# mrlooi/PoseCNN

Measured on AMD Instinct MI355X. Metric: frames/sec 640x480x21-class Hough-vote+RoI+ADD-loss, 1/2/4/8 MI355X, higher is better.
Workload: dtype f32 (FC GEMMs: exact 3-way split-bf16 x6 MFMA, products within 2^-24, fp32 accumulate: fp32-faithful)

## Files before the change

### include/posecnn_hip.h

```cpp
#ifndef POSECNN_HIP_H
#define POSECNN_HIP_H

#include <stddef.h>
#include <stdint.h>

#ifdef __cplusplus
extern "C" {
#endif

#define PCNN_OK 0
#define PCNN_EINVAL 1
#define PCNN_EHIP 2
#define PCNN_ECAPACITY 3

#define PCNN_MAX_ROI 128

int pcnn_abi_version(void);
const char* pcnn_strerror(int code);

int pcnn_set_completion_event(void* event);
int pcnn_completion_event_pending(void);

size_t pcnn_hough_voting_workspace_size(int B, int H, int W, int C, int skip_pixels, float vote_thr);

// ... 36 lines not shown
                           float scale_b, int B, int C, const float* rois, int R_cap, int roi_stride,
                           int batch_base, const int32_t* num_rois_dev, int pooled_h, int pooled_w, float* top_sum,
                           int32_t* argmax_a, int32_t* argmax_b, void* stream);

int pcnn_roi_pool_fwd_pair_px(const float* data_a, int Ha, int Wa, float scale_a, const float* data_b, int Hb,
                              int Wb, float scale_b, int B, int C, const float* rois, int R_cap, int roi_stride,
                              int batch_base, const int32_t* num_rois_dev, int pooled_h, int pooled_w,
                              float* top_sum, uint16_t* argmax_a, uint16_t* argmax_b, void* stream);

size_t pcnn_roi_pool_bwd_workspace_size(int B, int R_cap);

int pcnn_roi_pool_bwd_form(int B, int H, int W, int C, int layout, int pool_channel, int pooled_h, int pooled_w,
                           int R_cap, int px);

int pcnn_roi_pool_bwd(const float* top_diff, const int32_t* argmax, int B, int H, int W, int C, int layout,
                      const float* rois, int R_cap, int roi_stride, int batch_base, const int32_t* num_rois_dev,
                      float spatial_scale, int pooled_h, int pooled_w, int pool_channel, float* bottom_diff,
                      void* workspace, size_t workspace_bytes, void* stream);

int pcnn_roi_pool_bwd_px(const float* top_diff, const uint16_t* argmax_px, int B, int H, int W, int C,
                         const float* rois, int R_cap, int roi_stride, int batch_base, const int32_t* num_rois_dev,
                         float spatial_scale, int pooled_h, int pooled_w, float* bottom_diff, void* workspace,
                         size_t workspace_bytes, void* stream);

size_t pcnn_add_loss_workspace_size(int R_cap, int C, int P);
size_t pcnn_add_loss_stats_offset(int R_cap, int C, int P);

int pcnn_add_loss_fwd(const float* pred, const float* target, const float* weight, const float* points,
                      const float* symmetry, int R_cap, const int32_t* num_rois_dev, int C, int P, float margin,
                      int loss_norm_rows, const int32_t* loss_norm_rows_dev, float* loss, float* bottom_diff,
                      void* workspace, size_t workspace_bytes, void* stream);

int pcnn_add_loss_prep(const float* weight, const float* symmetry, int R_cap, const int32_t* num_rois_dev, int C,
                       int P, void* workspace, size_t workspace_bytes, void* stream);
int pcnn_add_loss_fwd_prepared(const float* pred, const float* target, const float* weight, const float* points,
                               const float* symmetry, int R_cap, const int32_t* num_rois_dev, int C, int P,
                               float margin, int loss_norm_rows, const int32_t* loss_norm_rows_dev, float* loss,
                               float* bottom_diff, void* workspace, size_t workspace_bytes, void* stream);

int pcnn_add_loss_fwd_head_bwd(const float* pred, const float* target, const float* weight, const float* points,
                               const float* symmetry, int R_cap, const int32_t* num_rois_dev, int C, int P,
                               float margin, int loss_norm_rows, const int32_t* loss_norm_rows_dev,
                               float* bottom_diff, void* workspace, size_t workspace_bytes, const float* tanh_out,
                               const float* d_pred_scale, float* d_y8, void* stream);
int pcnn_add_loss_total(int R_cap, const int32_t* num_rois_dev, int C, int P, const void* workspace,
                        size_t workspace_bytes, float* loss, void* stream);
// ... 197 lines not shown
```

### posecnn_amd/_lib.py

```python
import ctypes
import os
import threading

import torch

_HERE = os.path.dirname(os.path.abspath(__file__))
LIB_PATH = os.environ.get("POSECNN_HIP_LIB") or os.path.join(_HERE, "libposecnn_hip.so")

_lib = None
_lock = threading.Lock()

c_int = ctypes.c_int
c_float = ctypes.c_float
c_size_t = ctypes.c_size_t
c_void_p = ctypes.c_void_p

_SIGS = {
    "pcnn_abi_version": (c_int, []),
    "pcnn_strerror": (ctypes.c_char_p, [c_int]),
    "pcnn_set_completion_event": (c_int, [c_void_p]),
    "pcnn_completion_event_pending": (c_int, []),
    "pcnn_hough_voting_workspace_size": (c_size_t, [c_int, c_int, c_int, c_int, c_int, c_float]),
    "pcnn_hough_voting": (c_int, [c_void_p, c_void_p, c_void_p, c_void_p, c_int, c_void_p, c_int, c_int, c_int,
                                  c_int, c_int, c_int, c_int, c_int, c_float, c_int, c_float, c_float, c_int,
# ... 3 lines not shown
                                       c_int, c_int, c_int, c_int, c_int, c_int, c_int, c_float, c_int, c_float,
                                       c_float, c_int, c_void_p, c_void_p, c_void_p, c_void_p, c_void_p, c_void_p,
                                       c_int, c_void_p, c_void_p, c_size_t, c_void_p]),
    "pcnn_hough_voting_compact": (c_int, [c_void_p, c_void_p, c_void_p, c_void_p, c_int, c_void_p, c_int, c_int,
                                          c_int, c_int, c_int, c_int, c_int, c_int, c_float, c_int, c_float, c_float,
                                          c_int, c_void_p, c_void_p, c_void_p, c_void_p, c_void_p, c_void_p, c_int,
                                          c_void_p, c_void_p, c_size_t, c_void_p]),
    "pcnn_hough_voting_grad": (c_int, [c_void_p, c_void_p, c_int, c_int, c_int, c_int, c_void_p]),
    "pcnn_hough_voting_diag": (c_int, [c_void_p, c_int, c_int, c_int, c_int, c_int, c_float, c_void_p, c_void_p]),
    "pcnn_roi_pool_fwd": (c_int, [c_void_p, c_int, c_int, c_int, c_int, c_int, c_void_p, c_int, c_int, c_int,
                                  c_void_p, c_float, c_int, c_int, c_int, c_void_p, c_void_p, c_void_p]),
    "pcnn_roi_pool_fwd_accumulate": (c_int, [c_void_p, c_int, c_int, c_int, c_int, c_int, c_void_p, c_int, c_int,
                                             c_int, c_void_p, c_float, c_int, c_int, c_int, c_void_p, c_void_p, c_void_p]),
    "pcnn_roi_pool_fwd_pair": (c_int, [c_void_p, c_int, c_int, c_float, c_void_p, c_int, c_int, c_float, c_int, c_int,
                                       c_void_p, c_int, c_int, c_int, c_void_p, c_int, c_int, c_void_p, c_void_p,
                                       c_void_p, c_void_p]),
    "pcnn_roi_pool_fwd_pair_px": (c_int, [c_void_p, c_int, c_int, c_float, c_void_p, c_int, c_int, c_float, c_int,
                                          c_int, c_void_p, c_int, c_int, c_int, c_void_p, c_int, c_int, c_void_p,
                                          c_void_p, c_void_p, c_void_p]),
    "pcnn_roi_pool_bwd_workspace_size": (c_size_t, [c_int, c_int]),
    "pcnn_roi_pool_bwd_form": (c_int, [c_int, c_int, c_int, c_int, c_int, c_int, c_int, c_int, c_int, c_int]),
    "pcnn_roi_pool_bwd_px": (c_int, [c_void_p, c_void_p, c_int, c_int, c_int, c_int, c_void_p, c_int, c_int, c_int,
                                     c_void_p, c_float, c_int, c_int, c_void_p, c_void_p, c_size_t, c_void_p]),
    "pcnn_roi_pool_bwd": (c_int, [c_void_p, c_void_p, c_int, c_int, c_int, c_int, c_int, c_void_p, c_int, c_int,
                                  c_int, c_void_p, c_float, c_int, c_int, c_int, c_void_p, c_void_p, c_size_t, c_void_p]),
    "pcnn_add_loss_workspace_size": (c_size_t, [c_int, c_int, c_int]),
    "pcnn_add_loss_stats_offset": (c_size_t, [c_int, c_int, c_int]),
    "pcnn_add_loss_fwd": (c_int, [c_void_p, c_void_p, c_void_p, c_void_p, c_void_p, c_int, c_void_p, c_int, c_int,
                                  c_float, c_int, c_void_p, c_void_p, c_void_p, c_void_p, c_size_t, c_void_p]),
    "pcnn_add_loss_fwd_prepared": (c_int, [c_void_p, c_void_p, c_void_p, c_void_p, c_void_p, c_int, c_void_p, c_int, c_int,
                                  c_float, c_int, c_void_p, c_void_p, c_void_p, c_void_p, c_size_t, c_void_p]),
    "pcnn_add_loss_prep": (c_int, [c_void_p, c_void_p, c_int, c_void_p, c_int, c_int, c_void_p, c_size_t, c_void_p]),
    "pcnn_add_loss_fwd_head_bwd": (c_int, [c_void_p, c_void_p, c_void_p, c_void_p, c_void_p, c_int, c_void_p, c_int,
                                           c_int, c_float, c_int, c_void_p, c_void_p, c_void_p, c_size_t, c_void_p,
                                           c_void_p, c_void_p, c_void_p]),
    "pcnn_add_loss_total": (c_int, [c_int, c_void_p, c_int, c_int, c_void_p, c_size_t, c_void_p, c_void_p]),
    "pcnn_add_loss_bwd": (c_int, [c_void_p, c_void_p, c_int, c_void_p, c_int, c_void_p, c_void_p]),
    "pcnn_div_rn_check": (c_int, [c_void_p, c_float, c_int, c_int, c_void_p, c_void_p]),
    "pcnn_backproject_fwd": (c_int, [c_void_p, c_void_p, c_void_p, c_void_p, c_int, c_void_p, c_int, c_int, c_int,
                                     c_int, c_int, c_int, c_int, c_float, c_void_p, c_void_p, c_void_p, c_void_p]),
    "pcnn_backproject_bwd": (c_int, [c_void_p, c_void_p, c_void_p, c_int, c_int, c_int, c_int, c_int, c_int,
                                     c_void_p, c_void_p]),
    "pcnn_gemm_workspace_size": (c_size_t, [c_int, c_int, c_int, c_int, c_int]),
    "pcnn_gemm": (c_int, [c_int, c_int, c_int, c_void_p, c_void_p, c_int, c_int, c_void_p, c_int, c_int, c_void_p,
                          c_int, c_void_p, c_int, c_void_p, c_int, c_void_p, c_void_p, c_int, c_void_p, c_size_t,
                          c_void_p]),
# ... 223 lines not shown
```

### posecnn_amd/csrc/roi_plan.h

```cpp
#pragma once

namespace pcnn_roi {

#ifndef PCNN_RBW_NARROW
#define PCNN_RBW_NARROW 8192
#endif
#ifndef PCNN_RBW_TH
#define PCNN_RBW_TH 2
#endif
static_assert(PCNN_RBW_TH == 1 || PCNN_RBW_TH == 2, "the entry-list forms are 1x4 and 2x4");

constexpr int kBWaves = 1;
constexpr int kBChunk = 128 * kBWaves;
constexpr int kBTileW = 4;
constexpr int kBGroup = 16;
constexpr int kBBins = 49;
constexpr int kBCap = kBGroup * kBBins;

enum BwdForm { kBwdRejected = -1, kBwdGeneric = 0, kBwdEnt1x4 = 1, kBwdEnt2x4 = 2 };

struct BwdPlan {
  int form;
  int tbh;
};
// ... 5 lines not shown
inline int bwd_tile_h(int B, int H, int W, int C) {
  const long nchunk = ((long)C + kBChunk - 1) / kBChunk;
  const long wg24 = (long)B * (((long)H + 1) / 2) * (((long)W + 3) / 4) * nchunk;
  return wg24 < PCNN_RBW_NARROW ? 1 : PCNN_RBW_TH;
}

inline BwdPlan bwd_plan(int B, int H, int W, int C, int layout, int pool_channel, int pooled_h, int pooled_w,
                        int R_cap, int px) {
  BwdPlan p = {kBwdRejected, 0};
  if (B <= 0 || H <= 0 || W <= 0 || C <= 0 || pooled_h <= 0 || pooled_w <= 0 || R_cap < 0 ||
      (layout != 0 && layout != 1) || !map_below(H, W, C, 1l << 31))
    return p;
  const int tbh = bwd_tile_h(B, H, W, C);
  const long bins = (long)pooled_h * pooled_w;
  const bool ent = layout == 0 && !pool_channel && C % 2 == 0 && (long)pooled_h * tbh <= 32 &&
                   (long)pooled_w * kBTileW <= 32 && kBGroup * bins <= kBCap && map_below(H, W, C, 1l << 30) &&
                   R_cap <= ((1l << 29) - 1) / (bins * C);
  if (px && !(ent && (long)H * W < 0xFFFF)) return p;
  p.form = !ent ? kBwdGeneric : tbh == 1 ? kBwdEnt1x4 : kBwdEnt2x4;
  p.tbh = ent ? tbh : 0;
  return p;
}

}
```

### posecnn_amd/csrc/roi_pooling.hip

```cpp
#include "pcnn_common.h"
#include "roi_plan.h"
#include <math.h>
#include <cfloat>

namespace {


struct RoiGeo {
  int b, cls, sw, sh, ew, eh;
  float bin_h, bin_w;
};

__device__ __forceinline__ RoiGeo roi_geo(const float* __restrict__ rois, int r, int stride, int batch_base,
                                          float scale, int PH, int PW) {
  const float* o = rois + (size_t)r * stride;
  RoiGeo g;
  g.b = (int)o[0] - batch_base;
  const int c0 = stride == 5 ? 1 : 2;
  g.cls = stride == 5 ? 0 : (int)o[1];
  g.sw = (int)roundf(o[c0 + 0] * scale);
  g.sh = (int)roundf(o[c0 + 1] * scale);
  g.ew = (int)roundf(o[c0 + 2] * scale);
  g.eh = (int)roundf(o[c0 + 3] * scale);
  const int roi_w = max(g.ew - g.sw + 1, 1);
// ... 11 lines not shown

__device__ __forceinline__ void bin_bounds(const RoiGeo& g, int ph, int pw, int H, int W, int& hs, int& he, int& ws,
                                           int& we) {
  hs = (int)floorf((float)ph * g.bin_h);
  ws = (int)floorf((float)pw * g.bin_w);
  he = (int)ceilf((float)(ph + 1) * g.bin_h);
  we = (int)ceilf((float)(pw + 1) * g.bin_w);
  hs = min(max(hs + g.sh, 0), H);
  he = min(max(he + g.sh, 0), H);
  ws = min(max(ws + g.sw, 0), W);
  we = min(max(we + g.sw, 0), W);
}

__device__ __forceinline__ void bins_of_pixel(const RoiGeo& g, int h, int w, int PH, int PW, int& phs, int& phe,
                                              int& pws, int& pwe) {
  phs = (int)floorf((float)(h - g.sh) / g.bin_h);
  phe = (int)ceilf((float)(h - g.sh + 1) / g.bin_h);
  pws = (int)floorf((float)(w - g.sw) / g.bin_w);
  pwe = (int)ceilf((float)(w - g.sw + 1) / g.bin_w);
  phs = min(max(phs, 0), PH);
  phe = min(max(phe, 0), PH);
  pws = min(max(pws, 0), PW);
  pwe = min(max(pwe, 0), PW);
}

__device__ __forceinline__ void upd(float v, int idx, float& m, int& a) {
  if (v > m) { m = v; a = idx; }
}

constexpr int kXcds = 8;
constexpr int kRun = 9;
__device__ __forceinline__ bool fwd_item(int R, int nbins, int& r, int& bin) {
  const int id = blockIdx.x;
  const int x = id % kXcds, local = id / kXcds;
  const int lr = local / nbins;
  bin = local % nbins;
  r = ((lr / kRun) * kXcds + x) * kRun + lr % kRun;
  return r < R;
}
static inline unsigned fwd_grid(int R_cap, int nbins) {
  return (unsigned)(kXcds * ((R_cap + kXcds * kRun - 1) / (kXcds * kRun)) * kRun * nbins);
}

template <bool PX = false>
__device__ __forceinline__ void bin_max4(const float* __restrict__ data, int B, int H, int W, int C,
                                         const RoiGeo& g, int ph, int pw, int c, float4& m, int4& a) {
// ... 122 lines not shown
    const int ch = pool_channel ? g.cls : c;
    int hs, he, ws, we;
    bin_bounds(g, ph, pw, H, W, hs, he, ws, we);
    const bool empty = bad || (he <= hs) || (we <= ws) || ch < 0 || ch >= C;
    float maxval = empty ? 0.f : -FLT_MAX;
    int maxidx = -1;
    if (!empty) {
      const float* bd = data + (size_t)g.b * H * W * C;
      for (int h = hs; h < he; h++)
        for (int w = ws; w < we; w++) {
          const int bi = layout == 0 ? (h * W + w) * C + ch : (ch * H + h) * W + w;
          const float v = bd[bi];
          if (v > maxval) { maxval = v; maxidx = bi; }
        }
    }
    top[idx] = acc ? top[idx] + maxval : maxval;
    argmax[idx] = maxidx;
  }
}

__global__ void __launch_bounds__(1024) k_roi_prep(const float* __restrict__ rois, int R_cap, int stride,
                                                    int batch_base, const int32_t* __restrict__ num_rois_dev, int B,
                                                    float scale, int PH, int PW, int32_t* __restrict__ geo,
                                                    int32_t* __restrict__ lo, int32_t* __restrict__ hi) {
  __shared__ int slo[1024], shi[1024];
  const int R = rows_of(num_rois_dev, R_cap);
  const int nb = B < 1024 ? B : 1024;
  for (int b = threadIdx.x; b < nb; b += blockDim.x) {
    slo[b] = 0x7fffffff;
    shi[b] = -1;
  }
  __syncthreads();
  for (int r = threadIdx.x; r < R; r += blockDim.x) {
    const RoiGeo g = roi_geo(rois, r, stride, batch_base, scale, PH, PW);
    int32_t* o = geo + (size_t)r * 8;
    o[0] = g.b; o[1] = g.cls; o[2] = g.sw; o[3] = g.sh; o[4] = g.ew; o[5] = g.eh;
    o[6] = __float_as_int(g.bin_h);
    o[7] = __float_as_int(g.bin_w);
    if (g.b >= 0 && g.b < nb) {
      atomicMin(&slo[g.b], r);
      atomicMax(&shi[g.b], r);
    }
  }
  __syncthreads();
  for (int b = threadIdx.x; b < B; b += blockDim.x) {
    lo[b] = b < nb ? slo[b] : 0;
    hi[b] = b < nb ? shi[b] : -1;
  }
}

using pcnn_roi::kBWaves;
using pcnn_roi::kBChunk;
using pcnn_roi::kBGroup;
using pcnn_roi::kBCap;
constexpr int kBBatch = 8;

template <int kBTH, int kBTW, bool PX>
__global__ void __launch_bounds__(64 * kBWaves) k_roi_bwd_ent(const float* __restrict__ top_diff,
                                                               const void* __restrict__ argmax, int B, int H, int W,
                                                               int C, const int32_t* __restrict__ geo,
                                                               const int32_t* __restrict__ lo,
                                                               const int32_t* __restrict__ hi, int PH, int PW,
                                                               float* __restrict__ bottom) {
  constexpr int kBPix = kBTH * kBTW;
  __shared__ int2 ent[kBCap];
  __shared__ int sh_total;
  const int tiles_w = (W + kBTW - 1) / kBTW, tiles_h = (H + kBTH - 1) / kBTH;
  const int nchunk = (C + kBChunk - 1) / kBChunk;
  const int ipx = (int)((gridDim.x + 7) / 8);
  int id = (int)(blockIdx.x % 8) * ipx + (int)(blockIdx.x / 8);
  if (id >= B * tiles_w * tiles_h * nchunk) return;
  const int chunk = id % nchunk;
  id /= nchunk;
  const int t = id % (tiles_w * tiles_h), b = id / (tiles_w * tiles_h);
  const int h0 = (t / tiles_w) * kBTH, w0 = (t % tiles_w) * kBTW;
  const int th = min(kBTH, H - h0), tw = min(kBTW, W - w0);
  const int lane = pcnn::lane_id(), wave = threadIdx.x >> 6;
  const int c = chunk * kBChunk + 2 * threadIdx.x;
// ... 3 lines not shown
#pragma unroll
  for (int p = 0; p < kBPix; p++) {
    acc[p] = make_float2(0.f, 0.f);
    const int pix = (h0 + p / kBTW) * W + w0 + p % kBTW;
    expv[p] = PX ? pix : pix * C + c;
  }
  constexpr int kNext = PX ? 0 : 1;
  const int r0 = lo[b], r1 = hi[b];
  const __amdgpu_buffer_rsrc_t rs_t = __builtin_amdgcn_make_buffer_rsrc((void*)top_diff, (short)0, 0x7fffffff, 0x00020000);
  const __amdgpu_buffer_rsrc_t rs_a = __builtin_amdgcn_make_buffer_rsrc((void*)argmax, (short)0, 0x7fffffff, 0x00020000);
  const unsigned voff = cok ? (unsigned)c * 4u : 0x80000000u;
  const unsigned voff_a = cok ? (unsigned)c * (PX ? 2u : 4u) : 0x80000000u;
  for (int rb = r0; rb <= r1; rb += 64) {
    uint32_t rbits = 0;
    uint32_t cbits = 0;
    const int r = rb + lane;
    if (wave == 0 && r <= r1) {
      const int32_t* gg = geo + (size_t)r * 8;
      RoiGeo g;
      g.b = gg[0]; g.sw = gg[2]; g.sh = gg[3]; g.ew = gg[4]; g.eh = gg[5];
      g.bin_h = __int_as_float(gg[6]);
      g.bin_w = __int_as_float(gg[7]);
      if (g.b == b && g.sh <= h0 + th - 1 && g.eh >= h0 && g.sw <= w0 + tw - 1 && g.ew >= w0) {
        for (int i = 0; i < th; i++) {
          const int h = h0 + i;
          if (h < g.sh || h > g.eh) continue;
          int s0 = (int)floorf((float)(h - g.sh) / g.bin_h), e0 = (int)ceilf((float)(h - g.sh + 1) / g.bin_h);
          s0 = min(max(s0, 0), PH);
          e0 = min(max(e0, 0), PH);
          for (int ph = s0; ph < e0; ph++) rbits |= 1u << (ph * kBTH + i);
        }
        for (int j = 0; j < tw; j++) {
          const int w = w0 + j;
          if (w < g.sw || w > g.ew) continue;
          int s0 = (int)floorf((float)(w - g.sw) / g.bin_w), e0 = (int)ceilf((float)(w - g.sw + 1) / g.bin_w);
          s0 = min(max(s0, 0), PW);
          e0 = min(max(e0, 0), PW);
          for (int pw = s0; pw < e0; pw++) cbits |= 1u << (pw * kBTW + j);
        }
      }
    }
    const uint64_t hits = __ballot(rbits && cbits);
    for (int g0 = 0; g0 < 64; g0 += kBGroup) {
      if (wave == 0) {
        const uint64_t gm = hits & (((1ull << kBGroup) - 1) << g0);
        const bool mine = (gm >> lane) & 1;
        int cnt = 0;
        if (mine) {
          int nph = 0, npw = 0;
          for (int ph = 0; ph < PH; ph++) nph += ((rbits >> (ph * kBTH)) & ((1u << kBTH) - 1)) != 0;
          for (int pw = 0; pw < PW; pw++) npw += ((cbits >> (pw * kBTW)) & ((1u << kBTW) - 1)) != 0;
          cnt = nph * npw;
        }
        int off = cnt;
#pragma unroll
        for (int d = 1; d < 64; d <<= 1) {
          const int v = __shfl_up(off, d, 64);
          if (lane >= d) off += v;
        }
        if (lane == 63) sh_total = off;
        off -= cnt;
        if (mine) {
// ... 42 lines not shown
          }
        }
      };
      if (total > 0) {
        int2 myA, myB, avA[kBBatch], avB[kBBatch];
        float2 dvA[kBBatch], dvB[kBBatch];
        fetch(0, myA, avA, dvA);
        for (int e0 = 0; e0 < total; e0 += 2 * kBBatch) {
          if (e0 + kBBatch < total) fetch(e0 + kBBatch, myB, avB, dvB);
          accumulate(e0, myA, avA, dvA);
          if (e0 + 2 * kBBatch < total) fetch(e0 + 2 * kBBatch, myA, avA, dvA);
          if (e0 + kBBatch < total) accumulate(e0 + kBBatch, myB, avB, dvB);
        }
      }
      __syncthreads();
    }
  }
  if (cok) {
#pragma unroll
    for (int i = 0; i < kBTH; i++)
#pragma unroll
      for (int j = 0; j < kBTW; j++)
        if (i < th && j < tw) *(float2*)(bottom + (((size_t)b * H + h0 + i) * W + w0 + j) * C + c) = acc[i * kBTW + j];
  }
}

__global__ void k_roi_bwd_generic(const float* __restrict__ top_diff, const int32_t* __restrict__ argmax, int B,
                                  int H, int W, int C, int layout, const int32_t* __restrict__ geo, int PH, int PW,
                                  int pool_channel, const int32_t* __restrict__ lo, const int32_t* __restrict__ hi,
                                  float* __restrict__ bottom) {
  const long npix = (long)B * H * W;
  const int Co = pool_channel ? 1 : C;
  for (long pi = (long)blockIdx.x * blockDim.x + threadIdx.x; pi < npix; pi += (long)gridDim.x * blockDim.x) {
    const int w = (int)(pi % W), h = (int)((pi / W) % H), b = (int)(pi / ((long)W * H));
    const int r0 = lo[b], r1 = hi[b];
    for (int r = r0; r <= r1; r++) {
      const int32_t* gg = geo + (size_t)r * 8;
      RoiGeo g;
      g.b = gg[0]; g.cls = gg[1]; g.sw = gg[2]; g.sh = gg[3]; g.ew = gg[4]; g.eh = gg[5];
      g.bin_h = __int_as_float(gg[6]);
      g.bin_w = __int_as_float(gg[7]);
      if (g.b != b) continue;
      if (!(w >= g.sw && w <= g.ew && h >= g.sh && h <= g.eh)) continue;
      int phs, phe, pws, pwe;
      bins_of_pixel(g, h, w, PH, PW, phs, phe, pws, pwe);
      const int cb = pool_channel ? g.cls : 0, ce = pool_channel ? g.cls + 1 : C;
// ... 122 lines not shown
}

static int roi_pool_bwd(const float* top_diff, const void* argmax, bool px, int B, int H, int W, int C, int layout,
                        const float* rois, int R_cap, int roi_stride, int batch_base, const int32_t* num_rois_dev,
                        float spatial_scale, int pooled_h, int pooled_w, int pool_channel, float* bottom_diff,
                        void* workspace, size_t workspace_bytes, void* stream) {
  PCNN_REQUIRE(top_diff && argmax && rois && bottom_diff && workspace && B > 0 && H > 0 && W > 0 && C > 0);
  PCNN_REQUIRE(pooled_h > 0 && pooled_w > 0 && (layout == 0 || layout == 1) && R_cap >= 0);
  PCNN_REQUIRE(roi_stride >= 6 || (roi_stride == 5 && !pool_channel));
  PCNN_REQUIRE((long)H * W * C < (1l << 31));
  if (workspace_bytes < pcnn_roi_pool_bwd_workspace_size(B, R_cap)) return PCNN_ECAPACITY;
  const pcnn_roi::BwdPlan plan =
      pcnn_roi::bwd_plan(B, H, W, C, layout, pool_channel, pooled_h, pooled_w, R_cap, px ? 1 : 0);
  const bool aligned =
      (((uintptr_t)top_diff | (uintptr_t)bottom_diff) & 7) == 0 && ((uintptr_t)argmax & (px ? 3 : 7)) == 0;
  const bool vec = plan.form != pcnn_roi::kBwdGeneric && aligned;
  PCNN_REQUIRE(plan.form != pcnn_roi::kBwdRejected && (!px || vec));
  hipStream_t st = (hipStream_t)stream;
  pcnn::Carve cv(workspace);
  int32_t* lo = cv.take<int32_t>(B);
  int32_t* hi = cv.take<int32_t>(B);
  int32_t* geo = cv.take<int32_t>((size_t)(R_cap > 0 ? R_cap : 1) * 8);
  hipLaunchKernelGGL(k_roi_prep, dim3(1), dim3(1024), 0, st, rois, R_cap, roi_stride, batch_base, num_rois_dev,
                     B, spatial_scale, pooled_h, pooled_w, geo, lo, hi);
  if (vec) {
    constexpr int tbw = pcnn_roi::kBTileW;
    const int tbh = plan.tbh, nchunk = (C + kBChunk - 1) / kBChunk;
    const int tiles = ((H + tbh - 1) / tbh) * ((W + tbw - 1) / tbw);
    const unsigned nwg = (unsigned)((B * tiles * nchunk + 7) / 8 * 8);
#define PCNN_RBW(TH, PXV)                                                                                  \
  pcnn::launch_last(k_roi_bwd_ent<TH, tbw, PXV>, dim3(nwg), dim3(64 * kBWaves), 0, st, top_diff, argmax, B, H, W, C, \
                    geo, lo, hi, pooled_h, pooled_w, bottom_diff)
    if (tbh == 1) {
      if (px) PCNN_RBW(1, true); else PCNN_RBW(1, false);
    } else {
      if (px) PCNN_RBW(2, true); else PCNN_RBW(2, false);
    }
#undef PCNN_RBW
  } else {
    if (hipMemsetAsync(bottom_diff, 0, (size_t)B * H * W * C * sizeof(float), st) != hipSuccess) return PCNN_EHIP;
    const long npix = (long)B * H * W;
    const int blocks = (int)((npix + 255) / 256 < 8192 ? (npix + 255) / 256 : 8192);
    hipLaunchKernelGGL(k_roi_bwd_generic, dim3(blocks), dim3(256), 0, st, top_diff, (const int32_t*)argmax, B, H, W,
                       C, layout, geo, pooled_h, pooled_w, pool_channel, lo, hi, bottom_diff);
  }
  PCNN_CHECK_LAUNCH();
  return PCNN_OK;
}

extern "C" int pcnn_roi_pool_bwd(const float* top_diff, const int32_t* argmax, int B, int H, int W, int C, int layout,
                                 const float* rois, int R_cap, int roi_stride, int batch_base,
                                 const int32_t* num_rois_dev, float spatial_scale, int pooled_h, int pooled_w,
                                 int pool_channel, float* bottom_diff, void* workspace, size_t workspace_bytes, void* stream) {
  return roi_pool_bwd(top_diff, argmax, false, B, H, W, C, layout, rois, R_cap, roi_stride, batch_base, num_rois_dev,
                      spatial_scale, pooled_h, pooled_w, pool_channel, bottom_diff, workspace, workspace_bytes, stream);
}

extern "C" int pcnn_roi_pool_bwd_px(const float* top_diff, const uint16_t* argmax_px, int B, int H, int W, int C,
                                    const float* rois, int R_cap, int roi_stride, int batch_base,
                                    const int32_t* num_rois_dev, float spatial_scale, int pooled_h, int pooled_w,
                                    float* bottom_diff, void* workspace, size_t workspace_bytes, void* stream) {
  return roi_pool_bwd(top_diff, argmax_px, true, B, H, W, C, 0, rois, R_cap, roi_stride, batch_base, num_rois_dev,
                      spatial_scale, pooled_h, pooled_w, 0, bottom_diff, workspace, workspace_bytes, stream);
}
```

### posecnn_amd/pipeline.py

```python
import contextlib

import torch

from . import _lib
from . import pose_head as ph
from .hough_voting_gpu_layer import hough_voting_gpu_op as hv
from .roi_pooling_layer import roi_pooling_op as rp
from .average_distance_loss import average_distance_loss_op as adl
from .exchange import GradShard, RoiExchange

CAP = hv.CAPACITY
_nullctx = contextlib.nullcontext


class PoseStep:
    def __init__(self, B, H, W, num_classes, device, conv4_hw=None, conv5_hw=None, channels=512, units=4096,
                 is_train=1, skip_pixels=10, vote_threshold=-1.0, vote_percentage=0.02, margin=0.01,
                 global_batch=None, batch_base=0, weights=None, dist=None, backward=True, precision=2,
                 overlap_weight_grads=True, pixel_argmax=True, keep_prob=None, drop_seed=0x5EED, side_prep=True,
                 drop_in_reduce=True, pipeline=False, prefetch_at="loss", fuse_loss_tail=True,
                 defer_side_join=False, signal_forks=True, pool_at_tail=False, fuse_fc8=True):
        self.B, self.H, self.W, self.C = B, H, W, num_classes
        self.dev = device
        self.is_train, self.skip, self.vthr, self.vper, self.margin = is_train, skip_pixels, vote_threshold, \
# ... 478 lines not shown
        if defer:
            self._mid_covers_pre = (self._primed is not None and self._pool_pending is None and
                                    not torch.cuda.is_current_stream_capturing())
            if self._mid_covers_pre:
                side.wait_stream(self.pre_stream)
            if self._bump_drop_step and self._mid_covers_pre:
                with torch.cuda.stream(side):
                    self.drop_step.add_(1)
                self._bump_drop_step = False
            self._side_mid_ev.record(side)
        ev = self._arm_fork("fc7_dx") if side is not None else None
        with self._t("gemm_fc8_fc7_dx"):
            self._g("fc7_dx", self.dy7, w.w7, self.dy6, b_trans=1, mask=self.y6, M_dev=nr, **dk)
        ev = self._fork_taken(ev)
        with self._t("gemm_fc6_dw"):
            weight_grads("w6", x, self.dy6, CAP, K6, w.units, fork_ev=ev)
        with self._t("gemm_fc6_dx"):
            self._g("fc6_dx", self.dy6, w.w6, self.dx, b_trans=1, M_dev=nr)
        if self.prefetch_at == "tail":
            self._prefetch()
        self._issue_pending_pool()
        dxp = self.dx.view(CAP, 7, 7, self.Ch)
        with self._t("roi_pool_bwd"):
            rp.roi_pool_grad(conv5, h["box"], self.arg5, dxp, 7, 7, 1.0 / 16.0, 0, num_rois=nr, out=self.dconv5,
                             batch_base=self.batch_base)
            rp.roi_pool_grad(conv4, h["box"], self.arg4, dxp, 7, 7, 1.0 / 8.0, 0, num_rois=nr, out=self.dconv4,
                             batch_base=self.batch_base)
        if self._bump_drop_step:
            self.drop_step.add_(1)
            self._bump_drop_step = False
        if defer:
            self._side_done_ev.record(side)
            self._side_pending = True
        elif side is not None:
            main.wait_stream(side)

    def _g(self, name, A, B, C, **kw):
        self._timed_gemm(name, lambda: ph.gemm(A, B, C, precision=self.prec, checked=False, **kw))
        return C

    def _timed_gemm(self, name, launch):
        if self.gemm_timer is None:
            return launch()
        e0, e1 = torch.cuda.Event(enable_timing=True), torch.cuda.Event(enable_timing=True)
        e0.record()
        out = launch()
        e1.record()
        self.gemm_timer.setdefault(name, []).append((e0, e1))
        return out

# ... 59 lines not shown
```

### posecnn_amd/roi_pooling_layer/roi_pooling_op.py

```python
import torch

from .. import _lib


def roi_pool(bottom_data, bottom_rois, pooled_height, pooled_width, spatial_scale, pool_channel=0, name=None,
             num_rois=None, layout=0, out=None, accumulate=False, batch_base=0):
    _lib.require_gpu(bottom_data, bottom_rois)
    if bottom_data.dim() != 4:
        raise ValueError("data must be 4-dimensional")
    if bottom_rois.dim() != 2:
        raise ValueError("rois must be 2-dimensional")
    data = bottom_data.contiguous().float()
    rois = bottom_rois.contiguous().float()
    if layout == 0:
        B, H, W, C = data.shape
    else:
        B, C, H, W = data.shape
    R, stride = rois.shape
    Co = 1 if pool_channel else C
    shape = (R, pooled_height, pooled_width, Co) if layout == 0 else (R, Co, pooled_height, pooled_width)
    if out is None:
        if accumulate:
            raise ValueError("accumulate=True needs out=(top, argmax)")
        top = torch.empty(shape, dtype=torch.float32, device=data.device)
# ... 84 lines not shown
    if out is not None:
        _lib.require(out, torch.float32, shape=tuple(bottom_data.shape), name="roi_pool_grad: out")
    lib = _lib.load()
    ws = _lib.workspace(lib.pcnn_roi_pool_bwd_workspace_size(B, R), bottom_data.device, "roi_bwd")
    dd = out if out is not None else torch.empty(bottom_data.shape, dtype=torch.float32, device=bottom_data.device)
    if R == 0:
        rois = argmax = grad = ws
    if px:
        if layout != 0 or pool_channel:
            raise ValueError("a pixel-index argmax needs NHWC data and pool_channel 0")
        rc = lib.pcnn_roi_pool_bwd_px(_lib.ptr(grad), _lib.ptr(argmax), B, H, W, C,
                                      _lib.ptr(rois), R, stride, int(batch_base), _lib.ptr(num_rois),
                                      float(spatial_scale), int(pooled_height), int(pooled_width), _lib.ptr(dd),
                                      _lib.ptr(ws), ws.numel(), _lib.stream_ptr())
    else:
        rc = lib.pcnn_roi_pool_bwd(_lib.ptr(grad), _lib.ptr(argmax), B, H, W, C, layout,
                                   _lib.ptr(rois), R, stride, int(batch_base), _lib.ptr(num_rois),
                                   float(spatial_scale), int(pooled_height), int(pooled_width), int(pool_channel),
                                   _lib.ptr(dd), _lib.ptr(ws), ws.numel(), _lib.stream_ptr())
    _lib.check(rc, "roi_pool_grad")
    return dd


class RoiPoolFunction(torch.autograd.Function):

    @staticmethod
    def forward(ctx, data, rois, pooled_height, pooled_width, spatial_scale, pool_channel=0, layout=0):
        top, arg = roi_pool(data, rois, pooled_height, pooled_width, spatial_scale, pool_channel, layout=layout)
        ctx.save_for_backward(data, rois, arg)
        ctx.params = (pooled_height, pooled_width, spatial_scale, pool_channel, layout)
        return top, arg

    @staticmethod
    def backward(ctx, grad, _garg):
        data, rois, arg = ctx.saved_tensors
        ph, pw, sc, pc, layout = ctx.params
        return roi_pool_grad(data, rois, arg, grad, ph, pw, sc, pc, layout=layout), None, None, None, None, None, None
```

Baseline: 4625.

## Fuse paired RoI-pool backward into one region-tiled kernel with LDS accumulation

Adds a paired RoI-pool backward path that handles the conv5 and conv4 gradient maps in a single launch. Each block owns a 4x4 pixel region and a channel slab, builds a list of overlapping RoI bins in LDS, gathers argmax and top_diff with buffer loads (double-buffered), and accumulates into an LDS tile before writing it out once. One shared prep kernel computes the geometry for both scales. The aim is to cut launch count and scattered global traffic. The cost is extra complexity and a fallback to the two separate launches when the layout conditions are not met.

```diff
diff --git a/include/posecnn_hip.h b/include/posecnn_hip.h
--- a/include/posecnn_hip.h
+++ b/include/posecnn_hip.h
@@ -82,6 +82,17 @@
                          const float* rois, int R_cap, int roi_stride, int batch_base, const int32_t* num_rois_dev,
                          float spatial_scale, int pooled_h, int pooled_w, float* bottom_diff, void* workspace,
                          size_t workspace_bytes, void* stream);
+
+size_t pcnn_roi_pool_bwd_pair_workspace_size(int B, int R_cap);
+int pcnn_roi_pool_bwd_pair_px(const float* top_diff, const uint16_t* argmax_a, int Ha, int Wa, float scale_a,
+                              float* bottom_a, const uint16_t* argmax_b, int Hb, int Wb, float scale_b,
+                              float* bottom_b, int B, int C, const float* rois, int R_cap, int roi_stride,
+                              int batch_base, const int32_t* num_rois_dev, int pooled_h, int pooled_w,
+                              void* workspace, size_t workspace_bytes, void* stream);
+
+int pcnn_roi_pool_bwd_pair_plan(int B, int H, int W, int C, int pooled_h, int pooled_w, int R_cap,
+                                int32_t* plan_host);
+uint32_t pcnn_roi_pool_recip_u16(int W);
 
 size_t pcnn_add_loss_workspace_size(int R_cap, int C, int P);
 size_t pcnn_add_loss_stats_offset(int R_cap, int C, int P);
diff --git a/posecnn_amd/_lib.py b/posecnn_amd/_lib.py
--- a/posecnn_amd/_lib.py
+++ b/posecnn_amd/_lib.py
@@ -49,6 +49,12 @@
     "pcnn_roi_pool_bwd_form": (c_int, [c_int, c_int, c_int, c_int, c_int, c_int, c_int, c_int, c_int, c_int]),
     "pcnn_roi_pool_bwd_px": (c_int, [c_void_p, c_void_p, c_int, c_int, c_int, c_int, c_void_p, c_int, c_int, c_int,
                                      c_void_p, c_float, c_int, c_int, c_void_p, c_void_p, c_size_t, c_void_p]),
+    "pcnn_roi_pool_bwd_pair_workspace_size": (c_size_t, [c_int, c_int]),
+    "pcnn_roi_pool_bwd_pair_px": (c_int, [c_void_p, c_void_p, c_int, c_int, c_float, c_void_p, c_void_p, c_int, c_int,
+                                          c_float, c_void_p, c_int, c_int, c_void_p, c_int, c_int, c_int, c_void_p,
+                                          c_int, c_int, c_void_p, c_size_t, c_void_p]),
+    "pcnn_roi_pool_bwd_pair_plan": (c_int, [c_int, c_int, c_int, c_int, c_int, c_int, c_int, c_void_p]),
+    "pcnn_roi_pool_recip_u16": (ctypes.c_uint32, [c_int]),
     "pcnn_roi_pool_bwd": (c_int, [c_void_p, c_void_p, c_int, c_int, c_int, c_int, c_int, c_void_p, c_int, c_int,
                                   c_int, c_void_p, c_float, c_int, c_int, c_int, c_void_p, c_void_p, c_size_t, c_void_p]),
     "pcnn_add_loss_workspace_size": (c_size_t, [c_int, c_int, c_int]),
diff --git a/posecnn_amd/csrc/roi_plan.h b/posecnn_amd/csrc/roi_plan.h
--- a/posecnn_amd/csrc/roi_plan.h
+++ b/posecnn_amd/csrc/roi_plan.h
@@ -51,4 +51,45 @@
   return p;
 }
 
+
+constexpr int kRgnH = 4, kRgnW = 4;
+constexpr int kRgnWaves = 2;
+constexpr int kRgnCap = 512;
+constexpr int kRgnSlabUnit = 64;
+
+struct RgnPlan {
+  int ok;
+  int rh, rw, nw;
+  int regs_h, regs_w;
+  int nslab;
+  long items;
+  int lds_bytes;
+  unsigned w_recip;
+};
+
+inline unsigned recip_u16(int W) { return (unsigned)((1ull << 32) / (unsigned)W) + 1u; }
+
+constexpr int rgn_lds_bytes(int rh, int rw, int nw) {
+  return rh * rw * kRgnSlabUnit * nw * 4 + kRgnCap * 8 + 16;
 }
+
+inline RgnPlan rgn_plan(int B, int H, int W, int C, int pooled_h, int pooled_w, int R_cap) {
+  RgnPlan p = {};
+  if (bwd_plan(B, H, W, C, 0, 0, pooled_h, pooled_w, R_cap, 1).form <= kBwdGeneric) return p;
+  if (C % kRgnSlabUnit != 0 || W < 2) return p;
+  p.rh = kRgnH;
+  p.rw = kRgnW;
+  p.nw = C % (kRgnSlabUnit * 2) == 0 && kRgnWaves >= 2 ? 2 : 1;
+  if ((long)pooled_h * p.rh > 64 || (long)pooled_w * p.rw > 64) return p;
+  p.regs_h = (H + p.rh - 1) / p.rh;
+  p.regs_w = (W + p.rw - 1) / p.rw;
+  p.nslab = C / (kRgnSlabUnit * p.nw);
+  p.items = (long)B * p.regs_h * p.regs_w * p.nslab;
+  p.lds_bytes = rgn_lds_bytes(p.rh, p.rw, p.nw);
+  p.w_recip = recip_u16(W);
+  if (p.items > (1l << 30) || p.lds_bytes > 64 * 1024) return p;
+  p.ok = 1;
+  return p;
+}
+
+}
diff --git a/posecnn_amd/csrc/roi_pooling.hip b/posecnn_amd/csrc/roi_pooling.hip
--- a/posecnn_amd/csrc/roi_pooling.hip
+++ b/posecnn_amd/csrc/roi_pooling.hip
@@ -57,6 +57,26 @@
   phe = min(max(phe, 0), PH);
   pws = min(max(pws, 0), PW);
   pwe = min(max(pwe, 0), PW);
+}
+
+__device__ __forceinline__ void bins_of_coord(int x, int start, float bin, int P, int& s0, int& e0) {
+  s0 = (int)floorf((float)(x - start) / bin);
+  e0 = (int)ceilf((float)(x - start + 1) / bin);
+  s0 = min(max(s0, 0), P);
+  e0 = min(max(e0, 0), P);
+}
+
+template <int T, typename M>
+__device__ __forceinline__ M accept_bits(int x0, int n, int start, int end, float bin, int P) {
+  M bits = 0;
+  for (int i = 0; i < n; i++) {
+    const int x = x0 + i;
+    if (x < start || x > end) continue;
+    int s0, e0;
+    bins_of_coord(x, start, bin, P, s0, e0);
+    for (int p = s0; p < e0; p++) bits |= (M)1 << (p * T + i);
+  }
+  return bits;
 }
 
 __device__ __forceinline__ void upd(float v, int idx, float& m, int& a) {
@@ -225,7 +245,8 @@
 __global__ void __launch_bounds__(1024) k_roi_prep(const float* __restrict__ rois, int R_cap, int stride,
                                                     int batch_base, const int32_t* __restrict__ num_rois_dev, int B,
                                                     float scale, int PH, int PW, int32_t* __restrict__ geo,
-                                                    int32_t* __restrict__ lo, int32_t* __restrict__ hi) {
+                                                    int32_t* __restrict__ lo, int32_t* __restrict__ hi,
+                                                    float scale_b, int32_t* __restrict__ geo_b) {
   __shared__ int slo[1024], shi[1024];
   const int R = rows_of(num_rois_dev, R_cap);
   const int nb = B < 1024 ? B : 1024;
@@ -240,6 +261,13 @@
     o[0] = g.b; o[1] = g.cls; o[2] = g.sw; o[3] = g.sh; o[4] = g.ew; o[5] = g.eh;
     o[6] = __float_as_int(g.bin_h);
     o[7] = __float_as_int(g.bin_w);
+    if (geo_b) {
+      const RoiGeo q = roi_geo(rois, r, stride, batch_base, scale_b, PH, PW);
+      int32_t* ob = geo_b + (size_t)r * 8;
+      ob[0] = q.b; ob[1] = q.cls; ob[2] = q.sw; ob[3] = q.sh; ob[4] = q.ew; ob[5] = q.eh;
+      ob[6] = __float_as_int(q.bin_h);
+      ob[7] = __float_as_int(q.bin_w);
+    }
     if (g.b >= 0 && g.b < nb) {
       atomicMin(&slo[g.b], r);
       atomicMax(&shi[g.b], r);
@@ -257,6 +285,8 @@
 using pcnn_roi::kBGroup;
 using pcnn_roi::kBCap;
 constexpr int kBBatch = 8;
+constexpr int kRgnBatch = 8;
+constexpr int kRgnGroup = 4;
 
 template <int kBTH, int kBTW, bool PX>
 __global__ void __launch_bounds__(64 * kBWaves) k_roi_bwd_ent(const float* __restrict__ top_diff,
@@ -306,22 +336,8 @@
       g.bin_h = __int_as_float(gg[6]);
       g.bin_w = __int_as_float(gg[7]);
       if (g.b == b && g.sh <= h0 + th - 1 && g.eh >= h0 && g.sw <= w0 + tw - 1 && g.ew >= w0) {
-        for (int i = 0; i < th; i++) {
-          const int h = h0 + i;
-          if (h < g.sh || h > g.eh) continue;
-          int s0 = (int)floorf((float)(h - g.sh) / g.bin_h), e0 = (int)ceilf((float)(h - g.sh + 1) / g.bin_h);
-          s0 = min(max(s0, 0), PH);
-          e0 = min(max(e0, 0), PH);
-          for (int ph = s0; ph < e0; ph++) rbits |= 1u << (ph * kBTH + i);
-        }
-        for (int j = 0; j < tw; j++) {
-          const int w = w0 + j;
-          if (w < g.sw || w > g.ew) continue;
-          int s0 = (int)floorf((float)(w - g.sw) / g.bin_w), e0 = (int)ceilf((float)(w - g.sw + 1) / g.bin_w);
-          s0 = min(max(s0, 0), PW);
-          e0 = min(max(e0, 0), PW);
-          for (int pw = s0; pw < e0; pw++) cbits |= 1u << (pw * kBTW + j);
-        }
+        rbits = accept_bits<kBTH, uint32_t>(h0, th, g.sh, g.eh, g.bin_h, PH);
+        cbits = accept_bits<kBTW, uint32_t>(w0, tw, g.sw, g.ew, g.bin_w, PW);
       }
     }
     const uint64_t hits = __ballot(rbits && cbits);
@@ -410,6 +426,178 @@
 #pragma unroll
       for (int j = 0; j < kBTW; j++)
         if (i < th && j < tw) *(float2*)(bottom + (((size_t)b * H + h0 + i) * W + w0 + j) * C + c) = acc[i * kBTW + j];
+  }
+}
+
+struct RgnMap {
+  const uint16_t* argmax;
+  const int32_t* geo;
+  float* bottom;
+  int H, W, regs_w, regs;
+  unsigned w_recip;
+  int items, ipx;
+};
+using pcnn_roi::kRgnCap;
+
+template <int RH, int RW, int NW, int KB>
+__global__ void __launch_bounds__(64 * NW) k_roi_bwd_rgn(const float* __restrict__ top_diff, RgnMap m0, RgnMap m1,
+                                                          int B, int C, const int32_t* __restrict__ lo,
+                                                          const int32_t* __restrict__ hi, int PH, int PW) {
+  static_assert(RH <= 8 && RW <= 8 && KB % kRgnGroup == 0 && KB <= 64, "an entry packs its row and column masks into 8 bits each");
+  constexpr int CS = 64 * NW, kPix = RH * RW;
+  __shared__ __attribute__((aligned(16))) float acc[kPix * CS];
+  __shared__ int2 ent[kRgnCap];
+  __shared__ int sh_total, sh_more;
+  const int x = (int)(blockIdx.x % 8);
+  int local = (int)(blockIdx.x / 8);
+  const bool second = local >= m0.ipx;
+  if (second) local -= m0.ipx;
+  const RgnMap& m = second ? m1 : m0;
+  int id = x * m.ipx + local;
+  if (id >= m.items) return;
+  const int nslab = C / CS;
+  const int slab = id % nslab;
+  id /= nslab;
+  const int t = id % m.regs, b = id / m.regs;
+  const int H = m.H, W = m.W;
+  const int h0 = (t / m.regs_w) * RH, w0 = (t % m.regs_w) * RW;
+  const int rh = min(RH, H - h0), rw = min(RW, W - w0);
+  const int tid = threadIdx.x, lane = pcnn::lane_id();
+  const int wave = __builtin_amdgcn_readfirstlane(tid >> 6);
+  const int c0 = slab * CS;
+  const unsigned w_recip = m.w_recip;
+  const int32_t* __restrict__ geo = m.geo;
+  const __amdgpu_buffer_rsrc_t rs_t = __builtin_amdgcn_make_buffer_rsrc((void*)(top_diff + c0), (short)0, 0x7fffffff, 0x00020000);
+  const __amdgpu_buffer_rsrc_t rs_a = __builtin_amdgcn_make_buffer_rsrc((void*)(m.argmax + c0), (short)0, 0x7fffffff, 0x00020000);
+  const unsigned voff = (unsigned)tid * 4u, voff_a = (unsigned)tid * 2u;
+  float* const mine = acc + tid;
+  bool touched = false;
+  const int r0 = lo[b], r1 = hi[b];
+  for (int rb = r0; rb <= r1; rb += 64) {
+    const int r = rb + lane;
+    RoiGeo g = {};
+    bool meets = false;
+    if (r <= r1) {
+      const int4 ga = *(const int4*)(geo + (size_t)r * 8), gb = *(const int4*)(geo + (size_t)r * 8 + 4);
+      g.b = ga.x; g.sw = ga.z; g.sh = ga.w; g.ew = gb.x; g.eh = gb.y;
+      g.bin_h = __int_as_float(gb.z);
+      g.bin_w = __int_as_float(gb.w);
+      meets = g.b == b && g.sh <= h0 + rh - 1 && g.eh >= h0 && g.sw <= w0 + rw - 1 && g.ew >= w0;
+    }
+    if (__ballot(meets) == 0) continue;
+    if (!touched) {
+      for (int i = tid; i < kPix * CS / 4; i += 64 * NW) ((float4*)acc)[i] = make_float4(0.f, 0.f, 0.f, 0.f);
+      touched = true;
+    }
+    uint64_t rbits = 0;
+    uint64_t cbits = 0;
+    int cnt = 0, incl = 0;
+    if (wave == 0) {
+      if (meets) {
+        rbits = accept_bits<RH, uint64_t>(h0, rh, g.sh, g.eh, g.bin_h, PH);
+        cbits = accept_bits<RW, uint64_t>(w0, rw, g.sw, g.ew, g.bin_w, PW);
+        int nph = 0, npw = 0;
+        for (int ph = 0; ph < PH; ph++) nph += ((rbits >> (ph * RH)) & ((1u << RH) - 1)) != 0;
+        for (int pw = 0; pw < PW; pw++) npw += ((cbits >> (pw * RW)) & ((1u << RW) - 1)) != 0;
+        cnt = nph * npw;
+      }
+      incl = cnt;
+#pragma unroll
+      for (int d = 1; d < 64; d <<= 1) {
+        const int v = __shfl_up(incl, d, 64);
+        if (lane >= d) incl += v;
+      }
+    }
+    int done = 0;
+    int more;
+    do {
+      if (wave == 0) {
+        const bool take = cnt > 0 && incl > done && incl - done <= kRgnCap;
+        const int nd = pcnn::wave_max(take ? incl : done);
+        if (lane == 63) {
+          sh_total = nd - done;
+          sh_more = incl > nd;
+        }
+        if (take) {
+          int off = incl - cnt - done;
+          const int rbase = r * PH;
+          for (int ph = 0; ph < PH; ph++) {
+            const uint32_t rm = (uint32_t)(rbits >> (ph * RH)) & ((1u << RH) - 1);
+            if (!rm) continue;
+            for (int pw = 0; pw < PW; pw++) {
+              const uint32_t cm = (uint32_t)(cbits >> (pw * RW)) & ((1u << RW) - 1);
+              if (!cm) continue;
+              ent[off++] = make_int2(((rbase + ph) * PW + pw) * C, (int)(rm | (cm << 8)));
+            }
+          }
+        }
+        done = nd;
+      }
+      __syncthreads();
+      const int total = sh_total;
+      more = sh_more;
+      auto target = [&](unsigned a, uint32_t mk, unsigned& off) {
+        const uint32_t rm = mk & 0xFFu, cm = mk >> 8;
+        const unsigned row = __umulhi(a, w_recip);
+        const unsigned li = row - (unsigned)h0, lj = a - row * (unsigned)W - (unsigned)w0;
+        off = (li * RW + lj) * CS;
+        return li < (unsigned)RH && lj < (unsigned)RW && (((rm >> (li & 7u)) & (cm >> (lj & 7u))) & 1u) != 0;
+      };
+      auto fetch = [&](int e0, int2& my, unsigned (&av)[KB], float (&dv)[KB]) {
+        my = ent[min(e0 + (lane & (KB - 1)), total - 1)];
+#pragma unroll
+        for (int k = 0; k < KB; k++) {
+          const int so = __builtin_amdgcn_readlane(my.x, k) * 4;
+          av[k] = (unsigned)(uint16_t)__builtin_amdgcn_raw_buffer_load_b16(rs_a, voff_a, so >> 1, 0);
+          dv[k] = __builtin_bit_cast(float, __builtin_amdgcn_raw_buffer_load_b32(rs_t, voff, so, 0));
+        }
+      };
+      auto apply = [&](int e0, const int2& my, const unsigned (&av)[KB], const float (&dv)[KB]) {
+#pragma unroll
+        for (int k0 = 0; k0 < KB; k0 += kRgnGroup) {
+          if (e0 + k0 >= total) break;
+          unsigned off[kRgnGroup];
+          bool ok[kRgnGroup];
+          float was[kRgnGroup], sum[kRgnGroup];
+#pragma unroll
+          for (int g = 0; g < kRgnGroup; g++) {
+            ok[g] = target(av[k0 + g], (uint32_t)__builtin_amdgcn_readlane(my.y, k0 + g), off[g]) &&
+                    e0 + k0 + g < total;
+            was[g] = mine[ok[g] ? off[g] : 0u];
+          }
+#pragma unroll
+          for (int g = 0; g < kRgnGroup; g++) {
+            float base = was[g];
+#pragma unroll
+            for (int i = 0; i < g; i++)
+              if (ok[i] && off[i] == off[g]) base = sum[i];
+            sum[g] = base + dv[k0 + g];
+            if (ok[g]) mine[off[g]] = sum[g];
+          }
+        }
+      };
+      if (total > 0) {
+        int2 myA, myB;
+        unsigned avA[KB], avB[KB];
+        float dvA[KB], dvB[KB];
+        fetch(0, myA, avA, dvA);
+        for (int e0 = 0; e0 < total; e0 += 2 * KB) {
+          if (e0 + KB < total) fetch(e0 + KB, myB, avB, dvB);
+          apply(e0, myA, avA, dvA);
+          if (e0 + 2 * KB < total) fetch(e0 + 2 * KB, myA, avA, dvA);
+          if (e0 + KB < total) apply(e0 + KB, myB, avB, dvB);
+        }
+      }
+      __syncthreads();
+    } while (more);
+  }
+  float* const bo = m.bottom + (((size_t)b * H + h0) * W + w0) * C + c0;
+  for (int i = tid; i < kPix * CS / 4; i += 64 * NW) {
+    const int pix = i / (CS / 4), c4 = (i % (CS / 4)) * 4;
+    const int pi = pix / RW, pj = pix % RW;
+    if (pi < rh && pj < rw)
+      *(float4*)(bo + ((size_t)pi * W + pj) * C + c4) =
+          touched ? *(const float4*)(acc + pix * CS + c4) : make_float4(0.f, 0.f, 0.f, 0.f);
   }
 }
 
@@ -578,7 +766,7 @@
   int32_t* hi = cv.take<int32_t>(B);
   int32_t* geo = cv.take<int32_t>((size_t)(R_cap > 0 ? R_cap : 1) * 8);
   hipLaunchKernelGGL(k_roi_prep, dim3(1), dim3(1024), 0, st, rois, R_cap, roi_stride, batch_base, num_rois_dev,
-                     B, spatial_scale, pooled_h, pooled_w, geo, lo, hi);
+                     B, spatial_scale, pooled_h, pooled_w, geo, lo, hi, 0.f, (int32_t*)nullptr);
   if (vec) {
     constexpr int tbw = pcnn_roi::kBTileW;
     const int tbh = plan.tbh, nchunk = (C + kBChunk - 1) / kBChunk;
@@ -619,3 +807,72 @@
   return roi_pool_bwd(top_diff, argmax_px, true, B, H, W, C, 0, rois, R_cap, roi_stride, batch_base, num_rois_dev,
                       spatial_scale, pooled_h, pooled_w, 0, bottom_diff, workspace, workspace_bytes, stream);
 }
+
+extern "C" size_t pcnn_roi_pool_bwd_pair_workspace_size(int B, int R_cap) {
+  return pcnn_roi_pool_bwd_workspace_size(B, R_cap) +
+         pcnn::align_up((size_t)(R_cap > 0 ? R_cap : 1) * 8 * sizeof(int32_t), 256);
+}
+
+extern "C" int pcnn_roi_pool_bwd_pair_plan(int B, int H, int W, int C, int pooled_h, int pooled_w, int R_cap,
+                                           int32_t* plan_host) {
+  PCNN_REQUIRE(plan_host);
+  const pcnn_roi::RgnPlan p = pcnn_roi::rgn_plan(B, H, W, C, pooled_h, pooled_w, R_cap);
+  const int32_t v[8] = {p.ok, p.rh, p.rw, p.nw, p.regs_h, p.regs_w, p.nslab, p.lds_bytes};
+  for (int i = 0; i < 8; i++) plan_host[i] = v[i];
+  return PCNN_OK;
+}
+
+extern "C" uint32_t pcnn_roi_pool_recip_u16(int W) { return W > 1 ? pcnn_roi::recip_u16(W) : 0u; }
+
+extern "C" int pcnn_roi_pool_bwd_pair_px(const float* top_diff, const uint16_t* argmax_a, int Ha, int Wa, float scale_a,
+                                         float* bottom_a, const uint16_t* argmax_b, int Hb, int Wb, float scale_b,
+                                         float* bottom_b, int B, int C, const float* rois, int R_cap, int roi_stride,
+                                         int batch_base, const int32_t* num_rois_dev, int pooled_h, int pooled_w,
+                                         void* workspace, size_t workspace_bytes, void* stream) {
+  PCNN_REQUIRE(top_diff && argmax_a && argmax_b && bottom_a && bottom_b && rois && workspace);
+  PCNN_REQUIRE(B > 0 && C > 0 && Ha > 0 && Wa > 0 && Hb > 0 && Wb > 0 && pooled_h > 0 && pooled_w > 0 && R_cap >= 0);
+  PCNN_REQUIRE(roi_stride >= 5);
+  if (workspace_bytes < pcnn_roi_pool_bwd_pair_workspace_size(B, R_cap)) return PCNN_ECAPACITY;
+  const pcnn_roi::RgnPlan pa = pcnn_roi::rgn_plan(B, Ha, Wa, C, pooled_h, pooled_w, R_cap);
+  const pcnn_roi::RgnPlan pb = pcnn_roi::rgn_plan(B, Hb, Wb, C, pooled_h, pooled_w, R_cap);
+  const bool aligned = (((uintptr_t)bottom_a | (uintptr_t)bottom_b) & 15) == 0 && ((uintptr_t)top_diff & 3) == 0 &&
+                       (((uintptr_t)argmax_a | (uintptr_t)argmax_b) & 1) == 0;
+  if (!(pa.ok && pb.ok && aligned)) {
+    const hipEvent_t ev = pcnn::take_done_event();
+    const int rc = roi_pool_bwd(top_diff, argmax_a, true, B, Ha, Wa, C, 0, rois, R_cap, roi_stride, batch_base,
+                                num_rois_dev, scale_a, pooled_h, pooled_w, 0, bottom_a, workspace, workspace_bytes, stream);
+    pcnn::t_done_event = ev;
+    if (rc != PCNN_OK) return rc;
+    return roi_pool_bwd(top_diff, argmax_b, true, B, Hb, Wb, C, 0, rois, R_cap, roi_stride, batch_base, num_rois_dev,
+                        scale_b, pooled_h, pooled_w, 0, bottom_b, workspace, workspace_bytes, stream);
+  }
+  hipStream_t st = (hipStream_t)stream;
+  pcnn::Carve cv(workspace);
+  int32_t* lo = cv.take<int32_t>(B);
+  int32_t* hi = cv.take<int32_t>(B);
+  int32_t* geo_a = cv.take<int32_t>((size_t)(R_cap > 0 ? R_cap : 1) * 8);
+  int32_t* geo_b = cv.take<int32_t>((size_t)(R_cap > 0 ? R_cap : 1) * 8);
+  hipLaunchKernelGGL(k_roi_prep, dim3(1), dim3(1024), 0, st, rois, R_cap, roi_stride, batch_base, num_rois_dev, B,
+                     scale_a, pooled_h, pooled_w, geo_a, lo, hi, scale_b, geo_b);
+  auto map_of = [](const pcnn_roi::RgnPlan& p, const uint16_t* argmax, const int32_t* geo, float* bottom, int H, int W) {
+    RgnMap m;
+    m.argmax = argmax; m.geo = geo; m.bottom = bottom;
+    m.H = H; m.W = W; m.regs_w = p.regs_w; m.regs = p.regs_h * p.regs_w;
+    m.w_recip = p.w_recip;
+    m.items = (int)p.items;
+    m.ipx = (int)((p.items + 7) / 8);
+    return m;
+  };
+  const RgnMap ma = map_of(pa, argmax_a, geo_a, bottom_a, Ha, Wa), mb = map_of(pb, argmax_b, geo_b, bottom_b, Hb, Wb);
+  using pcnn_roi::kRgnH;
+  using pcnn_roi::kRgnW;
+  const unsigned grid = 8u * (unsigned)(ma.ipx + mb.ipx);
+  if (pa.nw == 2)
+    pcnn::launch_last(k_roi_bwd_rgn<kRgnH, kRgnW, 2, kRgnBatch>, dim3(grid), dim3(128), 0, st, top_diff, ma, mb, B, C,
+                      lo, hi, pooled_h, pooled_w);
+  else
+    pcnn::launch_last(k_roi_bwd_rgn<kRgnH, kRgnW, 1, kRgnBatch>, dim3(grid), dim3(64), 0, st, top_diff, ma, mb, B, C,
+                      lo, hi, pooled_h, pooled_w);
+  PCNN_CHECK_LAUNCH();
+  return PCNN_OK;
+}
diff --git a/posecnn_amd/pipeline.py b/posecnn_amd/pipeline.py
--- a/posecnn_amd/pipeline.py
+++ b/posecnn_amd/pipeline.py
@@ -524,10 +524,14 @@
         self._issue_pending_pool()
         dxp = self.dx.view(CAP, 7, 7, self.Ch)
         with self._t("roi_pool_bwd"):
-            rp.roi_pool_grad(conv5, h["box"], self.arg5, dxp, 7, 7, 1.0 / 16.0, 0, num_rois=nr, out=self.dconv5,
-                             batch_base=self.batch_base)
-            rp.roi_pool_grad(conv4, h["box"], self.arg4, dxp, 7, 7, 1.0 / 8.0, 0, num_rois=nr, out=self.dconv4,
-                             batch_base=self.batch_base)
+            if self.arg5.dtype == torch.int16:
+                rp.roi_pool_grad_pair(conv5, 1.0 / 16.0, conv4, 1.0 / 8.0, h["box"], self.arg5, self.arg4, dxp, 7, 7,
+                                      num_rois=nr, out=(self.dconv5, self.dconv4), batch_base=self.batch_base)
+            else:
+                rp.roi_pool_grad(conv5, h["box"], self.arg5, dxp, 7, 7, 1.0 / 16.0, 0, num_rois=nr, out=self.dconv5,
+                                 batch_base=self.batch_base)
+                rp.roi_pool_grad(conv4, h["box"], self.arg4, dxp, 7, 7, 1.0 / 8.0, 0, num_rois=nr, out=self.dconv4,
+                                 batch_base=self.batch_base)
         if self._bump_drop_step:
             self.drop_step.add_(1)
             self._bump_drop_step = False
diff --git a/posecnn_amd/roi_pooling_layer/roi_pooling_op.py b/posecnn_amd/roi_pooling_layer/roi_pooling_op.py
--- a/posecnn_amd/roi_pooling_layer/roi_pooling_op.py
+++ b/posecnn_amd/roi_pooling_layer/roi_pooling_op.py
@@ -130,6 +130,46 @@
     return dd
 
 
+def roi_pool_grad_pair(data_a, scale_a, data_b, scale_b, rois, argmax_a, argmax_b, grad, pooled_height, pooled_width,
+                       num_rois=None, out=None, batch_base=0):
+    _lib.require_gpu(data_a, data_b, rois, argmax_a, argmax_b, grad)
+    if data_a.dim() != 4 or data_b.dim() != 4 or rois.dim() != 2:
+        raise ValueError("data must be 4-dimensional and rois 2-dimensional")
+    B, Ha, Wa, C = data_a.shape
+    Bb, Hb, Wb, Cb = data_b.shape
+    if (Bb, Cb) != (B, C):
+        raise ValueError("both maps need the same batch and channel count")
+    rois = rois.contiguous().float()
+    R, stride = rois.shape
+    if stride < 5:
+        raise ValueError(f"roi_pool_grad_pair: rois rows need at least 5 columns, got {stride}")
+    if argmax_a.dtype != torch.int16 or argmax_b.dtype != torch.int16:
+        raise ValueError("roi_pool_grad_pair: the argmax tensors must be int16 (pixel index)")
+    n_top = R * int(pooled_height) * int(pooled_width) * C
+    argmax_a, argmax_b, grad = argmax_a.contiguous(), argmax_b.contiguous(), grad.contiguous().float()
+    if argmax_a.numel() != n_top or argmax_b.numel() != n_top or grad.numel() != n_top:
+        raise ValueError(f"roi_pool_grad_pair: argmax and grad must have {n_top} elements "
+                         f"(R x pooled_height x pooled_width x channels), got {argmax_a.numel()}, "
+                         f"{argmax_b.numel()} and {grad.numel()}")
+    _lib.require_counter(num_rois, "roi_pool_grad_pair: num_rois")
+    if out is None:
+        out = (torch.empty(data_a.shape, dtype=torch.float32, device=data_a.device),
+               torch.empty(data_b.shape, dtype=torch.float32, device=data_b.device))
+    da, db = out
+    _lib.require(da, torch.float32, shape=tuple(data_a.shape), name="roi_pool_grad_pair: out[0]")
+    _lib.require(db, torch.float32, shape=tuple(data_b.shape), name="roi_pool_grad_pair: out[1]")
+    lib = _lib.load()
+    ws = _lib.workspace(lib.pcnn_roi_pool_bwd_pair_workspace_size(B, R), data_a.device, "roi_bwd_pair")
+    if R == 0:
+        rois = argmax_a = argmax_b = grad = ws
+    rc = lib.pcnn_roi_pool_bwd_pair_px(_lib.ptr(grad), _lib.ptr(argmax_a), Ha, Wa, float(scale_a), _lib.ptr(da),
+                                       _lib.ptr(argmax_b), Hb, Wb, float(scale_b), _lib.ptr(db), B, C, _lib.ptr(rois),
+                                       R, stride, int(batch_base), _lib.ptr(num_rois), int(pooled_height),
+                                       int(pooled_width), _lib.ptr(ws), ws.numel(), _lib.stream_ptr())
+    _lib.check(rc, "roi_pool_grad_pair")
+    return da, db
+
+
 class RoiPoolFunction(torch.autograd.Function):
 
     @staticmethod
```

Result: no change. 4642 (median of 2 runs) (+0.4%).
